# aexoden/snesimage

Measured on AMD Instinct MI355X. Metric: candidate palettes scored/sec, higher is better.
Workload: dtype f32

## Files before the change

snesimage_amd/csrc/kernels.hpp:

```cpp
#pragma once
#include "color.hpp"

namespace snes {

constexpr int kMaxScales = SSIM2_NUM_SCALES;
constexpr int kBlurRadius = 5;

SNES_HD long long idx_c4(int x, int y, int H) { return ((long long)(x >> 2) * H + y) * 4 + (x & 3); }
SNES_HD long long idx_r4(int x, int y, int W) { return ((long long)(y >> 2) * W + x) * 4 + (y & 3); }
SNES_HD long long idx_xt4(int x, int y, int H) { return ((((long long)(x >> 6) * (H >> 2)) + (y >> 2)) << 8) + ((x & 63) << 2) + (y & 3); }

struct BlurK {
    float n2[3];
    float d1[3];
};

struct Geom {
    int W, H, nscales;
    int sw[kMaxScales], sh[kMaxScales];
    int th[kMaxScales];
    long long off_xyb[kMaxScales], off_xybT[kMaxScales], off_hout[kMaxScales];
    long long cand_stride;
    long long src_off[kMaxScales];
};
// ... 318 lines not shown
            float v[3];
            const int o4 = down_odd_row(G, 5, by) - 2 * by;
            for (int c = 0; c < 3; c++) { float sum = 0.0f; sum += l4[c][0][0]; sum += l4[c][0][1]; sum += l4[c][o4][0]; sum += l4[c][o4][1]; v[c] = sum * 0.25f; }
            float X, Y, B;
            linear_to_positive_xyb(v[0], v[1], v[2], X, Y, B);
            if (by >= G.th[5]) X = Y = B = 0.0f;
            size_t ns = (size_t)WS * HS;
            float *o = wbase + (CAND ? G.off_xyb[5] : G.src_off[5]);
            float *oT = CAND ? (wbase + G.off_xybT[5]) : (P.workT + G.src_off[5]);
            o[(size_t)by * WS + bx] = X; o[ns + (size_t)by * WS + bx] = Y; o[2 * ns + (size_t)by * WS + bx] = B;
            oT[(size_t)bx * HS + by] = X; oT[ns + (size_t)bx * HS + by] = Y; oT[2 * ns + (size_t)bx * HS + by] = B;
        }
    }
#undef SNES_DOWN_LEVEL
}

__global__ __launch_bounds__(256) void k_source_scale0(const uint8_t *__restrict__ orig, const float *__restrict__ eotf, int W, int H,
                                                       float *__restrict__ lin0, float *__restrict__ img1, float *__restrict__ img1T) {
    int px = blockIdx.x * blockDim.x + threadIdx.x;
    if (px >= W * H) return;
    int x = px % W, y = px / W;
    uint32_t o = reinterpret_cast<const uint32_t *>(orig)[px];
    float r = eotf[o & 0xff], g = eotf[(o >> 8) & 0xff], b = eotf[(o >> 16) & 0xff];
    size_t n = (size_t)W * H;
    lin0[px] = r; lin0[n + px] = g; lin0[2 * n + px] = b;
    float X, Y, B;
    linear_to_positive_xyb(r, g, b, X, Y, B);
    img1[px] = X; img1[n + px] = Y; img1[2 * n + px] = B;
    size_t pt = (size_t)x * H + y;
    img1T[pt] = X; img1T[n + pt] = Y; img1T[2 * n + pt] = B;
}

__device__ __forceinline__ void maps_accumulate(double (&acc)[6], float m1, float sd1, float a1, double r1, float m2, float v22, float v12, float i2) {
    const float mu22 = m2 * m2, mu12 = m1 * m2;
    const float mu_diff = m1 - m2;
    const float num_m = fmaf(mu_diff, -mu_diff, 1.0f);
    const float num_s = fmaf(2.0f, v12 - mu12, SSIM2_C2);
    const float denom_s = sd1 + (v22 - mu22) + SSIM2_C2;
    double d = 1.0 - (double)((num_m * num_s) / denom_s);
    d = d > 0.0 ? d : 0.0;
    acc[0] += d;
    const double dd = d * d;
    acc[1] += dd * dd;
    const double d1 = ((double)fabsf(i2 - m2) - (double)a1) * r1;
    const double art = d1 > 0.0 ? d1 : 0.0;
    const double det = (-d1) > 0.0 ? (-d1) : 0.0;
    acc[2] += art;
    const double a2 = art * art;
    acc[3] += a2 * a2;
    acc[4] += det;
    const double l2 = det * det;
    acc[5] += l2 * l2;
}
__device__ __forceinline__ float source_sd1(float mu1, float sigma11) { const float mu11 = mu1 * mu1; return sigma11 - mu11; }
__device__ __forceinline__ float source_a1(float img1, float mu1) { return fabsf(img1 - mu1); }
__device__ __forceinline__ double source_r1(float a1) { return 1.0 / (1.0 + (double)a1); }
__global__ __launch_bounds__(256) void k_src_pad_rows(Geom G, float *__restrict__ sd1, double *__restrict__ r1) {
    const int s = (int)blockIdx.y;
    if (s >= G.nscales) return;
    const int W = G.sw[s], pad = G.sh[s] - G.th[s];
    const int n = 3 * W * pad;
    for (int i = (int)(blockIdx.x * blockDim.x + threadIdx.x); i < n; i += (int)(gridDim.x * blockDim.x)) {
        const int c = i / (W * pad), rem = i - c * (W * pad);
        const size_t idx = (size_t)G.src_off[s] + (size_t)c * W * G.sh[s] + (size_t)G.th[s] * W + rem;
        sd1[idx] = __builtin_nanf("");
        r1[idx] = 0.0;
    }
}

struct HParams {
    Geom G; BlurK K;
    int s, npairs, ncol, perceptual, use_maps, sub_size;
    const unsigned long long *packT; const float *pal_xyb; const float *cand_tab; const float *cand_lab; const float *labpxT;
    const float *in1T;
    const float *in2T;
    float *work;
    const uint8_t *mapsT; const uint8_t *tile_pal;
};

template <bool S0, bool PERCEPTUAL>
__global__ __launch_bounds__(256) void k_hpass(HParams P) {
    __shared__ __attribute__((aligned(16))) float buf[3][256][20];
    __shared__ float s_lut[3][256];
    const Geom &G = P.G;
    const int s = P.s;
    const int W = G.sw[s], H = G.sh[s];
    const int t = threadIdx.x;
    const int ppw = 256 / H;
    const int ql = t / H, y = t - ql * H;
    const int pair_raw = blockIdx.x * ppw + ql;
    const bool active = ql < ppw && pair_raw < P.npairs;
    const int pair = active ? pair_raw : 0;
    const int cand = pair / 3, ch = pair - cand * 3;
    const size_t ns = (size_t)W * H;

    float cand_v = 0.0f; uint32_t crgb = 0; Lab cl; cl.l = cl.a = cl.b = 0.0f; uint32_t cand_slot_ci = 0xffffffffu;
    if (S0) {
        for (int i = t; i < 3 * 256; i += 256) { int c = i >> 8, j = i & 255; s_lut[c][j] = (j < P.ncol + 2) ? P.pal_xyb[3 * j + c] : 0.0f; }
        cand_v = P.cand_tab[8 * (size_t)cand + 3 + ch];
        crgb = __float_as_uint(P.cand_tab[8 * (size_t)cand + 6]);
        cand_slot_ci = __float_as_uint(P.cand_tab[8 * (size_t)cand + 7]);
        if (PERCEPTUAL) { cl.l = P.cand_lab[3 * cand]; cl.a = P.cand_lab[3 * cand + 1]; cl.b = P.cand_lab[3 * cand + 2]; }
        __syncthreads();
    }
    const float *in1 = P.in1T + (size_t)ch * ns;
    const float *in2 = S0 ? nullptr : (P.in2T ? P.in2T + (size_t)ch * ns : P.work + (size_t)cand * G.cand_stride + G.off_xybT[s] + (size_t)ch * ns);
// ... 279 lines not shown
```

snesimage_amd/csrc/kernels_sparse.hpp:

```cpp
#pragma once
#include "kernels.hpp"

namespace snes {

constexpr int kGroupsTotal = 126;

struct CandMeta {
    int ngroups[kMaxScales];
    int xmin;
    int won;
    unsigned char glist[kGroupsTotal + 2];
    short gslot[kGroupsTotal];
    unsigned char gcb[kGroupsTotal];
};
__device__ __forceinline__ int item_k(unsigned int it) { return (int)(it >> 14); }
__device__ __forceinline__ int item_g(unsigned int it) { return (int)((it >> 8) & 63u); }
__device__ __forceinline__ int item_j(unsigned int it) { return (int)((it >> 2) & 63u); }
__device__ __forceinline__ int item_ch(unsigned int it) { return (int)(it & 3u); }
constexpr int kColBuckets = 4;
constexpr int kItemLists = kMaxScales * kColBuckets;

struct SparseGeom {
    long long off_lin[kMaxScales], off_xybC[kMaxScales], off_xybR[kMaxScales], off_hout[kMaxScales];
    long long cand_stride;
// ... 844 lines not shown
                if (P.perceptual && !is_base) {
                    const int px0 = y * W + (g << 2);
                    const uint32_t b4 = (P.bitmap[(size_t)k * (G.W * G.H / 32) + (px0 >> 5)] >> (px0 & 31)) & 0xfu;
                    c0 = (b4 & 1u) ? (uint32_t)P.ncol : (c_pa.x >> 24); c1 = (b4 & 2u) ? (uint32_t)P.ncol : (c_pa.z >> 24);
                    c2 = (b4 & 4u) ? (uint32_t)P.ncol : (c_pb.x >> 24); c3 = (b4 & 8u) ? (uint32_t)P.ncol : (c_pb.z >> 24);
                } else {
                    c0 = sparse_ci(c_pa.x, c_pa.y & never, crgb, (uint32_t)P.ncol); c1 = sparse_ci(c_pa.z, c_pa.w & never, crgb, (uint32_t)P.ncol);
                    c2 = sparse_ci(c_pb.x, c_pb.y & never, crgb, (uint32_t)P.ncol); c3 = sparse_ci(c_pb.z, c_pb.w & never, crgb, (uint32_t)P.ncol);
                }
                r2[u].x = c0 == (uint32_t)P.ncol ? cand_v : s_lut[ch][c0]; r2[u].y = c1 == (uint32_t)P.ncol ? cand_v : s_lut[ch][c1];
                r2[u].z = c2 == (uint32_t)P.ncol ? cand_v : s_lut[ch][c2]; r2[u].w = c3 == (uint32_t)P.ncol ? cand_v : s_lut[ch][c3];
            }
            const float v1[4] = {r1[u].x, r1[u].y, r1[u].z, r1[u].w}, v2[4] = {r2[u].x, r2[u].y, r2[u].z, r2[u].w};
            const float l1[4] = {r1[ua].z, r1[ua].w, r1[ub].x, r1[ub].y}, l2[4] = {r2[ua].z, r2[ua].w, r2[ub].x, r2[ub].y};
            float outp[3][4];
#pragma unroll
            for (int q = 0; q < 4; q++) {
                const float s0 = l2[q] + v2[q];
                const float s1 = (l2[q] * l2[q]) + (v2[q] * v2[q]);
                const float s2 = (l1[q] * l2[q]) + (v1[q] * v2[q]);
                if ((q & 1) == 0) { SNES_HSTEP(s0, sa[0], sb[0], outp[0][q]) SNES_HSTEP(s1, sa[1], sb[1], outp[1][q]) SNES_HSTEP(s2, sa[2], sb[2], outp[2][q]) }
                else { SNES_HSTEP(s0, sb[0], sa[0], outp[0][q]) SNES_HSTEP(s1, sb[1], sa[1], outp[1][q]) SNES_HSTEP(s2, sb[2], sa[2], outp[2][q]) }
            }
            if (g >= 1) {
#pragma unroll
                for (int p = 0; p < 3; p++) {
                    s_tr[p][lane * 5 + 0] = outp[p][0]; s_tr[p][lane * 5 + 1] = outp[p][1]; s_tr[p][lane * 5 + 2] = outp[p][2]; s_tr[p][lane * 5 + 3] = outp[p][3];
                }
                __syncthreads();
                const int x = ((g - 1) << 2) + li;
                const size_t o = ((size_t)(x >> 6) << 8) + ((size_t)(x & 63) << 2);
                if (valid) {
#pragma unroll
                    for (int p = 0; p < 3; p++) {
                        float4 v;
                        v.x = s_tr[p][(k4 + 0) * 5 + li]; v.y = s_tr[p][(k4 + 1) * 5 + li]; v.z = s_tr[p][(k4 + 2) * 5 + li]; v.w = s_tr[p][(k4 + 3) * 5 + li];
                        *reinterpret_cast<float4 *>(out + (size_t)p * 4 * W + o) = v;
                    }
                }
                __syncthreads();
            }
        }
    }
    }
}

template <bool UNI, int S0M, int BM>
__device__ __forceinline__ void sparse_v_body(const SparseParams &P, const int s) {
    __shared__ float s_lut[256];
    __shared__ short s_gslot[256];
    __shared__ __attribute__((aligned(16))) unsigned char s_raw[(2 + 3) * 3 * 256 * sizeof(float2)];
    float2 (*s_xy)[3][256] = reinterpret_cast<float2 (*)[3][256]>(s_raw);
    float2 (*s_zw)[3][256] = reinterpret_cast<float2 (*)[3][256]>(s_raw + 2 * 3 * 256 * sizeof(float2));
    double (*red)[6] = reinterpret_cast<double (*)[6]>(s_raw);
    static_assert(sizeof(s_raw) >= 256 * 6 * sizeof(double), "reduction scratch must fit the tail ring");
    const Geom &G = P.G;
    if (s >= G.nscales) return;
    const int W = G.sw[s], H = G.sh[s];
    const bool S0 = S0M == 2 ? s == 0 : S0M == 1;
    const int t = threadIdx.x;
    const int ppw = 256 / W;
    const bool is_base = BM == 2 ? P.is_base != 0 : BM == 1;
    const int npairs = is_base ? 3 : P.ncand * 3;
    if ((int)blockIdx.x * ppw >= npairs) return;
    const int ql = t / W, x = t - ql * W;
    const int pair_raw = blockIdx.x * ppw + ql;
    const bool active = pair_raw < npairs;
    const int pair = active ? pair_raw : 0;
    const int k = is_base ? P.base : P.k0 + (P.order ? P.order[pair / 3] : pair / 3), ch = pair % 3;
    if (S0) {
        s_lut[t] = (t < P.ncol + 2) ? P.pal_xyb[3 * t + ch] : 0.0f;
    }
    const size_t ns = (size_t)W * H;
    const int H4 = H >> 2;
    const CandMeta *M = P.meta + k;
    for (int i = t; i < ppw * H4; i += 256) {
        const int pr = blockIdx.x * ppw + i / H4;
        const int pq = (pr < npairs ? pr : 0) / 3;
        const int kk = is_base ? P.base : P.k0 + (P.order ? P.order[pq] : pq);
        s_gslot[i] = (P.meta + kk)->gslot[P.S.goff[s] + i % H4];
    }
    __syncthreads();
    const short *gslot = s_gslot + ql * H4;
    const int ng = M->ngroups[s];
    const int cmin = (M->xmin >> s) - 5;
    const bool skip = !is_base && (ng == 0 || x <= cmin);
    int gs = skip ? H4 + 1 : (is_base ? 0 : (int)M->glist[P.S.goff[s]]);
    if (UNI) {
        const int gs_pair = is_base ? 0 : (ng == 0 ? H4 + 1 : (int)M->glist[P.S.goff[s]]);
        gs = __builtin_amdgcn_readfirstlane(__all(skip) ? H4 + 1 : gs_pair);
    }
#define SNES_GSLOT(I) (UNI ? __builtin_amdgcn_readfirstlane((int)gslot[I]) : (int)gslot[I])
    const float cand_v = is_base ? 0.0f : P.cand_tab[8 * (size_t)k + 3 + ch];
    const uint32_t crgb = is_base ? 0u : __float_as_uint(P.cand_tab[8 * (size_t)k + 6]);
    const uint32_t never = is_base ? 0u : 0xffffffffu;
    const float *mine = P.store + (size_t)k * P.S.cand_stride;
    const float *basep = P.store + (size_t)P.base * P.S.cand_stride;
    const size_t hx = ((size_t)(x >> 6) << 6) + (size_t)(x & 63);
    const float4 *hb = reinterpret_cast<const float4 *>(basep + P.S.off_hout[s]) + (size_t)(ch * 3) * W + hx;
    const float4 *hm = reinterpret_cast<const float4 *>(mine + P.S.off_hout[s]) + (size_t)(ch * 3) * W + hx;
    const float4 *xb = S0 ? nullptr : reinterpret_cast<const float4 *>(basep + P.S.off_xybR[s]) + (size_t)ch * W + x;
    const float4 *xm = S0 ? nullptr : reinterpret_cast<const float4 *>(mine + P.S.off_xybR[s]) + (size_t)ch * W + x;
    const float4 *mu1 = reinterpret_cast<const float4 *>(P.mu1R4 + G.src_off[s] + (size_t)ch * ns) + x;
    const float4 *sd1 = reinterpret_cast<const float4 *>(P.sd1R4 + G.src_off[s] + (size_t)ch * ns) + x;
    const float4 *a1 = reinterpret_cast<const float4 *>(P.a1R4 + G.src_off[s] + (size_t)ch * ns) + x;
    const double2 *r1 = reinterpret_cast<const double2 *>(P.r1R4 + G.src_off[s] + (size_t)ch * ns) + 2 * (size_t)x;
    const uint4 *pk = S0 ? reinterpret_cast<const uint4 *>(P.packR4) + 2 * (size_t)x : nullptr;
    float *ckf = P.ckf + P.S.off_ckf[s] + (size_t)ch * (H4 + 2) * 18 * W + x;
    double *cka = P.cka + P.S.off_cka[s] + (size_t)ch * (H4 + 2) * 6 * W + x;

    const float n2_0 = P.K.n2[0], n2_1 = P.K.n2[1], n2_2 = P.K.n2[2];
    const float d1_0 = P.K.d1[0], d1_1 = P.K.d1[1], d1_2 = P.K.d1[2];
    float sa[3][3], sb[3][3];
    double acc[6];
    if (is_base) {
#pragma unroll
        for (int p = 0; p < 3; p++)
#pragma unroll
            for (int q = 0; q < 3; q++) { sa[p][q] = 0.0f; sb[p][q] = 0.0f; }
#pragma unroll
        for (int q = 0; q < 6; q++) acc[q] = 0.0;
    } else {
        const float *cf = ckf + (size_t)gs * 18 * W;
        const double *ca = cka + (size_t)gs * 6 * W;
#pragma unroll
        for (int p = 0; p < 3; p++)
#pragma unroll
            for (int q = 0; q < 3; q++) { sa[p][q] = cf[(size_t)(p * 6 + q) * W]; sb[p][q] = cf[(size_t)(p * 6 + 3 + q) * W]; }
#pragma unroll
        for (int q = 0; q < 6; q++) acc[q] = ca[(size_t)q * W];
    }
    const int W9 = 9 * W, W3 = 3 * W;
    auto hgroup = [&](int g) -> const float4 * {
        const int sl = SNES_GSLOT(g);
        return sl >= 0 ? hm + (uint32_t)__mul24(sl, W9) : hb + (uint32_t)__mul24(g, W9);
    };
    auto hload = [&](int g, int p) -> float4 { return hgroup(g)[(uint32_t)__mul24(p, W)]; };
    const float4 zero4 = make_float4(0.f, 0.f, 0.f, 0.f);
    float4 bufA[3], bufB[3];
#pragma unroll
    for (int p = 0; p < 3; p++) {
        float4 g1 = zero4, g2 = zero4, g3 = zero4;
        bufA[p] = zero4; bufB[p] = zero4;
        if (UNI ? gs <= H4 : !skip) {
            if (gs < H4) bufA[p] = hload(gs, p);
            if (gs - 1 >= 0) g1 = hload(gs - 1, p);
            if (gs - 2 >= 0) g2 = hload(gs - 2, p);
            if (gs - 3 >= 0) g3 = hload(gs - 3, p);
        }
        s_xy[1][p][t] = make_float2(g1.x, g1.y); s_zw[2][p][t] = make_float2(g1.z, g1.w);
        s_xy[0][p][t] = make_float2(g2.x, g2.y); s_zw[1][p][t] = make_float2(g2.z, g2.w);
        s_zw[0][p][t] = make_float2(g3.z, g3.w);
    }
    const int gm0 = gs >= 1 ? gs - 1 : 0;
    const float4 *p_m1 = mu1 + (uint32_t)__mul24(gm0, W), *p_sd1 = sd1 + (uint32_t)__mul24(gm0, W), *p_a1 = a1 + (uint32_t)__mul24(gm0, W);
    const double2 *p_r1 = r1 + 2u * (uint32_t)__mul24(gm0, W);
    const uint4 *p_pk = S0 ? pk + 2u * (uint32_t)__mul24(gm0, W) : nullptr;
    const uint32_t *bm = (S0 && P.perceptual && !is_base) ? P.bitmap + (size_t)k * (G.W * G.H / 32) : nullptr;
    float4 n_m1 = zero4, n_sd1 = zero4, n_a1 = zero4, n_x = zero4;
    double2 n_ra = make_double2(1.0, 1.0), n_rb = n_ra;
    uint4 n_pa = make_uint4(0, 0, 0, 0), n_pb = n_pa;
    float *ck_f = BM == 1 ? ckf + (size_t)gs * 18 * W : nullptr;
    double *ck_a = BM == 1 ? cka + (size_t)gs * 6 * W : nullptr;
#define SNES_VGROUP(U, CUR, NXT)                                                                                              \
    {                                                                                                                         \
        const int g = g0 + (U);                                                                                               \
        if (g > H4) break;                                                                                                    \
// ... 26 lines not shown
                if (S0) { n_pa = p_pk[0]; n_pb = p_pk[1]; p_pk += 2 * W; }                                                    \
                else n_x = xb[(uint32_t)__mul24(g, W3)];                                                                      \
            }                                                                                                                 \
        } else if (g >= 1) {                                                                                                  \
            c_m1 = *p_m1; c_sd1 = *p_sd1; c_a1 = *p_a1; c_ra = p_r1[0]; c_rb = p_r1[1];                                       \
            p_m1 += W; p_sd1 += W; p_a1 += W; p_r1 += 2 * W;                                                                  \
            if (S0) { c_pa = p_pk[0]; c_pb = p_pk[1]; p_pk += 2 * W; }                                                        \
            else { const int sl = SNES_GSLOT(g - 1); c_x = sl >= 0 ? xm[(uint32_t)__mul24(sl, W3)] : xb[(uint32_t)__mul24(g - 1, W3)]; } \
        }                                                                                                                     \
        float outp[3][4];                                                                                                     \
        _Pragma("unroll") for (int p = 0; p < 3; p++) {                                                                       \
            const float2 tz = s_zw[(U) % 3][p][t], tx = s_xy[(U) % 2][p][t];       \
            s_zw[(U) % 3][p][t] = make_float2(CUR[p].z, CUR[p].w);                                                            \
            s_xy[(U) % 2][p][t] = make_float2(CUR[p].x, CUR[p].y);                                                            \
            SNES_VSTEP(tz.x + CUR[p].x, sa[p], sb[p], outp[p][0])                                                             \
            SNES_VSTEP(tz.y + CUR[p].y, sb[p], sa[p], outp[p][1])                                                             \
            SNES_VSTEP(tx.x + CUR[p].z, sa[p], sb[p], outp[p][2])                                                             \
            SNES_VSTEP(tx.y + CUR[p].w, sb[p], sa[p], outp[p][3])                                                             \
        }                                                                                                                     \
        if (g >= 1) {                                                                                                         \
            float i2v[4] = {c_x.x, c_x.y, c_x.z, c_x.w};                                                                      \
            if (S0) {                                                                                                         \
                uint32_t c0, c1, c2, c3;                                                                                      \
                if (is_base || SNES_GSLOT(g - 1) < 0) {  \
                    c0 = c_pa.x >> 24; c1 = c_pa.z >> 24; c2 = c_pb.x >> 24; c3 = c_pb.z >> 24;                               \
                } else if (bm) {                                                       \
                    const int px0 = ((g - 1) << 2) * W + x;                                                                   \
                    c0 = won_bit(bm, px0) ? (uint32_t)P.ncol : (c_pa.x >> 24); c1 = won_bit(bm, px0 + W) ? (uint32_t)P.ncol : (c_pa.z >> 24);               \
                    c2 = won_bit(bm, px0 + 2 * W) ? (uint32_t)P.ncol : (c_pb.x >> 24); c3 = won_bit(bm, px0 + 3 * W) ? (uint32_t)P.ncol : (c_pb.z >> 24);   \
                } else {                                                                                                      \
                    c0 = sparse_ci(c_pa.x, c_pa.y & never, crgb, (uint32_t)P.ncol); c1 = sparse_ci(c_pa.z, c_pa.w & never, crgb, (uint32_t)P.ncol);         \
                    c2 = sparse_ci(c_pb.x, c_pb.y & never, crgb, (uint32_t)P.ncol); c3 = sparse_ci(c_pb.z, c_pb.w & never, crgb, (uint32_t)P.ncol);         \
                }                                                                                                             \
                i2v[0] = c0 == (uint32_t)P.ncol ? cand_v : s_lut[c0]; i2v[1] = c1 == (uint32_t)P.ncol ? cand_v : s_lut[c1];   \
                i2v[2] = c2 == (uint32_t)P.ncol ? cand_v : s_lut[c2]; i2v[3] = c3 == (uint32_t)P.ncol ? cand_v : s_lut[c3];   \
            }                                                                                                                 \
            const float m1v[4] = {c_m1.x, c_m1.y, c_m1.z, c_m1.w}, sd1v[4] = {c_sd1.x, c_sd1.y, c_sd1.z, c_sd1.w}, a1v[4] = {c_a1.x, c_a1.y, c_a1.z, c_a1.w}; \
            const double r1v[4] = {c_ra.x, c_ra.y, c_rb.x, c_rb.y};                                                           \
            _Pragma("unroll") for (int q = 0; q < 4; q++)                                                                     \
                maps_accumulate(acc, m1v[q], sd1v[q], a1v[q], r1v[q], outp[0][q], outp[1][q], outp[2][q], i2v[q]);            \
        }                                                                                                                     \
    }
    for (int g0 = gs; g0 <= H4; g0 += 6) {
        SNES_VGROUP(0, bufA, bufB) SNES_VGROUP(1, bufB, bufA) SNES_VGROUP(2, bufA, bufB)
        SNES_VGROUP(3, bufB, bufA) SNES_VGROUP(4, bufA, bufB) SNES_VGROUP(5, bufB, bufA)
    }
#undef SNES_VGROUP
#undef SNES_GSLOT
    if (is_base && active) {
        double *ca = cka + (size_t)(H4 + 1) * 6 * W;
#pragma unroll
        for (int q = 0; q < 6; q++) ca[(size_t)q * W] = acc[q];
    }
    __syncthreads();
#pragma unroll
    for (int q = 0; q < 6; q++) red[t][q] = active ? acc[q] : 0.0;
    __syncthreads();
    for (int stride = W >> 1; stride > 0; stride >>= 1) {
        if (x < stride) {
#pragma unroll
            for (int q = 0; q < 6; q++) red[t][q] += red[t + stride][q];
        }
        __syncthreads();
    }
    if (x == 0 && active) {
        double *o = P.part + (((size_t)k * G.nscales + s) * 3 + ch) * 6;
#pragma unroll
        for (int q = 0; q < 6; q++) o[q] = red[t][q];
    }
}
__global__ __launch_bounds__(256, 2) void k_sparse_v(SparseParams P) { sparse_v_body<false, 2, 2>(P, (int)blockIdx.y + P.s_first); }
__device__ __forceinline__ void sparse_v_base_body(const SparseParams &P) {
    const int s = (int)blockIdx.y;
    if (s >= P.G.nscales) return;
    if (P.G.sw[s] >= 64) sparse_v_body<true, 0, 1>(P, s);
    else sparse_v_body<false, 0, 1>(P, s);
}
#undef SNES_HSTEP
#undef SNES_VSTEP

__device__ __forceinline__ void build_plist_body(const unsigned long long *__restrict__ pack, int npx, uint4 *__restrict__ plist, int *__restrict__ count) {
    const int px = blockIdx.x * blockDim.x + threadIdx.x;
    unsigned long long w = 0;
    if (px < npx) w = pack[px];
    const uint32_t thr = (uint32_t)(w >> 32);
    const bool hit = thr != 0u;
    const unsigned long long m = __ballot(hit);
    if (m == 0ull) return;
    const int lane = threadIdx.x & 63, leader = __ffsll((long long)m) - 1;
    int base = 0;
    if (lane == leader) base = atomicAdd(count, __popcll(m));
    base = __shfl(base, leader);
    if (hit) plist[base + __popcll(m & ((1ull << lane) - 1ull))] = make_uint4((uint32_t)px, (uint32_t)w & 0x00ffffffu, thr, 0u);
}

__global__ __launch_bounds__(256) void k_remap_fill4(MapsParams P) {
    const int q = blockIdx.x * 256 + threadIdx.x;
    if (q * 4 >= P.npx) return;
    const uint4 a = reinterpret_cast<const uint4 *>(P.pack)[2 * (size_t)q], b = reinterpret_cast<const uint4 *>(P.pack)[2 * (size_t)q + 1];
    const uint32_t lo[4] = {a.x, a.z, b.x, b.z};
    uint32_t word = 0;
#pragma unroll
    for (int i = 0; i < 4; i++) {
        const uint32_t ci0 = lo[i] >> 24;
        word |= (ci0 == (uint32_t)P.ncol ? (uint32_t)P.si : (ci0 == (uint32_t)P.ncol + 1u ? 0u : ci0 % (uint32_t)P.sub_size)) << (8 * i);
    }
    const int c0 = blockIdx.y * kRemapCands;
    for (int cc = 0; cc < kRemapCands && c0 + cc < P.ncand; cc++) reinterpret_cast<uint32_t *>(P.maps + (size_t)(c0 + cc) * P.npx)[q] = word;
}
__global__ __launch_bounds__(256) void k_remap_won_lab(MapsParams P, const uint4 *__restrict__ plist, const int *__restrict__ plist_count) {
    __shared__ uint32_t s_queue[4][128];
    const int lane = threadIdx.x & 63, w = threadIdx.x >> 6;
    const int cand = (int)blockIdx.x;
    if (cand >= P.ncand) return;
    Lab cl; cl.l = P.cand_lab[3 * cand]; cl.a = P.cand_lab[3 * cand + 1]; cl.b = P.cand_lab[3 * cand + 2];
    const float cch = sqrtf(cl.a * cl.a + cl.b * cl.b);
    uint8_t *map = P.maps + (size_t)cand * P.npx;
    const int n = *plist_count;
    auto full_test = [&](int i) {
        const uint4 e = plist[i];
        Lab t; t.l = P.labpx[3 * (size_t)e.x]; t.a = P.labpx[3 * (size_t)e.x + 1]; t.b = P.labpx[3 * (size_t)e.x + 2];
// ... 59 lines not shown
```

snesimage_amd/csrc/kernels_sparse2.hpp:

```cpp
#pragma once
#include "kernels_sparse.hpp"
#include "kernels_fast.hpp"

namespace snes {

#define SNES_HSTEP(SUM, A, B, OUT)                                                   \
    {                                                                                \
        float o1_ = (SUM) * n2_0, o3_ = (SUM) * n2_1, o5_ = (SUM) * n2_2;            \
        o1_ = fmaf(-1.0f, B[0], o1_); o3_ = fmaf(-1.0f, B[1], o3_); o5_ = fmaf(-1.0f, B[2], o5_); \
        o1_ = fmaf(mp_0, A[0], o1_); o3_ = fmaf(mp_1, A[1], o3_); o5_ = fmaf(mp_2, A[2], o5_);    \
        B[0] = o1_; B[1] = o3_; B[2] = o5_;                                          \
        OUT = o1_ + o3_ + o5_;                                                       \
    }
#define SNES_VSTEP(SUM, A, B, OUT)                                                   \
    {                                                                                \
        float o1_ = fmaf(A[0], d1_0, B[0]), o3_ = fmaf(A[1], d1_1, B[1]), o5_ = fmaf(A[2], d1_2, B[2]); \
        o1_ = fmaf((SUM), n2_0, -o1_); o3_ = fmaf((SUM), n2_1, -o3_); o5_ = fmaf((SUM), n2_2, -o5_);    \
        B[0] = o1_; B[1] = o3_; B[2] = o5_;                                          \
        OUT = o1_ + o3_ + o5_;                                                       \
    }

struct H2Shared {
    __attribute__((aligned(16))) float out[16 * (4 * 32 + 4)];
    long long hbase[16], xbase[16];
// ... 280 lines not shown
                    const int im_ = 2 * m + half;                                                                             \
                    fv[m] = *reinterpret_cast<const float4 *>(s_out + im_ * ISTR + fl * 4);                                   \
                    fb[m] = (fp == 3) ? s_xbase[im_] : s_hbase[im_];                                                          \
                }                                                                                                             \
                _Pragma("unroll") for (int m = 0; m < 2; m++) {                                                               \
                    float *dst = (fb[m] >= 0 && fl < NP * 8) ? P.store + fb[m] + o_l : trash;                                 \
                    *reinterpret_cast<float4 *>(dst) = fv[m];                                                                 \
                }                                                                                                             \
                asm volatile("" ::: "memory");                                                                               \
            }                                                                                                                 \
        }
        { const int g = gs; SNES_H2Q_ITER(0, false, false) }
        for (int g0 = gs + 1; g0 <= G4; g0 += 6) {
            { const int g = g0; SNES_H2Q_ITER(1, true, false) }
            { const int g = g0 + 1; if (g > G4) break; SNES_H2Q_ITER(2, true, true) }
            { const int g = g0 + 2; if (g > G4) break; SNES_H2Q_ITER(3, true, false) }
            { const int g = g0 + 3; if (g > G4) break; SNES_H2Q_ITER(4, true, true) }
            { const int g = g0 + 4; if (g > G4) break; SNES_H2Q_ITER(5, true, false) }
            { const int g = g0 + 5; if (g > G4) break; SNES_H2Q_ITER(6, true, true) }
        }
#undef SNES_H2Q_ITER
    }
}
template <bool BASE>
__device__ __forceinline__ void sparse_h2q_dispatch(const SparseParams &P, const int list, const int bx, const int gx) {
    const int s = list / kColBuckets;
    if (s >= P.G.nscales || P.G.sw[s] < 64 || (list % kColBuckets) >= (P.G.sw[s] >> 6)) return;
    __shared__ H2Shared sh;
    if (s == 0) sparse_h2q_body<true, BASE>(P, list, bx, gx, sh); else sparse_h2q_body<false, BASE>(P, list, bx, gx, sh);
}

__device__ __forceinline__ int uni(int v) { return __builtin_amdgcn_readfirstlane(v); }
template <typename T> __device__ __forceinline__ T ld_at(const void *sbase, uint32_t voff) { return *reinterpret_cast<const T *>(reinterpret_cast<const char *>(sbase) + voff); }
typedef __amdgpu_buffer_rsrc_t rsrc_t;
typedef unsigned int u32x4 __attribute__((ext_vector_type(4)));
__device__ __forceinline__ rsrc_t make_rsrc(const void *p) {
    const unsigned long long a = (unsigned long long)p;
    const unsigned long long u = ((unsigned long long)(uint32_t)__builtin_amdgcn_readfirstlane((int)(a >> 32)) << 32) | (uint32_t)__builtin_amdgcn_readfirstlane((int)a);
    return __builtin_amdgcn_make_buffer_rsrc(reinterpret_cast<void *>(u), 0, 0x7fffffff, 0x00020000);
}
__device__ __forceinline__ float4 buf_ld4(rsrc_t r, uint32_t voff, uint32_t soff) {
    const u32x4 v = __builtin_amdgcn_raw_buffer_load_b128(r, (int)voff, (int)soff, 0);
    return make_float4(__uint_as_float(v.x), __uint_as_float(v.y), __uint_as_float(v.z), __uint_as_float(v.w));
}
__device__ __forceinline__ double2 buf_ld2d(rsrc_t r, uint32_t voff, uint32_t soff) {
    const u32x4 v = __builtin_amdgcn_raw_buffer_load_b128(r, (int)voff, (int)soff, 0);
    return make_double2(__hiloint2double((int)v.y, (int)v.x), __hiloint2double((int)v.w, (int)v.z));
}

template <bool BASE>
__device__ __forceinline__ void sparse_v2_body(const SparseParams &P, const int s, const int bx) {
    __shared__ short s_slot[4][64];
    __shared__ __attribute__((aligned(16))) unsigned char s_raw[(2 + 3) * 3 * 256 * sizeof(float2)];
    double (*red)[6] = reinterpret_cast<double (*)[6]>(s_raw);
    static_assert(sizeof(s_raw) >= 256 * 6 * sizeof(double), "reduction scratch must fit the tail ring");
    const Geom &G = P.G;
    const int W = uni(G.sw[s]), H = uni(G.sh[s]), H4 = H >> 2;
    const int t = threadIdx.x, lane = t & 63;
    const int wv = uni(t >> 6);
    const int wpp = W >> 6, ppw = 4 / wpp;
    const int npairs = BASE ? 3 : P.ncand * 3;
    if (bx * ppw >= npairs) return;
    const int ql = wv / wpp, xw = (wv - ql * wpp) << 6;
    const int pair_raw = bx * ppw + ql;
    const bool active = pair_raw < npairs;
    const int pair = active ? pair_raw : 0;
    const int ch = BASE ? pair : pair / P.ncand, ci = BASE ? 0 : pair - ch * P.ncand;
    const int k = BASE ? P.base : uni(P.k0 + (P.order ? P.order[ci] : ci));
    const CandMeta *M = P.meta + k;
    int gs;
    {
        const int g = lane;
        short sl = -1;
        if (!BASE && g < H4) { sl = M->gslot[P.S.goff[s] + g]; if (sl >= 0 && ((int)M->gcb[P.S.goff[s] + g] << 6) > xw) sl = -1; }
        s_slot[wv][lane] = sl;
        const unsigned long long own = __ballot(sl >= 0);
        gs = BASE ? 0 : uni(own ? __ffsll((long long)own) - 1 : H4 + 1);
    }
    __syncthreads();

    const size_t ns = (size_t)W * H;
    const float *store_k = P.store + (size_t)k * P.S.cand_stride, *store_b = P.store + (size_t)P.base * P.S.cand_stride;
    const rsrc_t h_own = make_rsrc(store_k + P.S.off_hout[s] + (size_t)(ch * 3) * 4 * W + ((size_t)(xw >> 6) << 8));
    const rsrc_t h_b = make_rsrc(store_b + P.S.off_hout[s] + (size_t)(ch * 3) * 4 * W + ((size_t)(xw >> 6) << 8));
    const rsrc_t h_zero = make_rsrc(P.zeros);
    const rsrc_t x_own = make_rsrc(store_k + P.S.off_xybR[s] + (size_t)ch * 4 * W + (size_t)xw * 4);
    const rsrc_t x_b = make_rsrc(store_b + P.S.off_xybR[s] + (size_t)ch * 4 * W + (size_t)xw * 4);
    const rsrc_t m1_b = make_rsrc(P.mu1R4 + G.src_off[s] + (size_t)ch * ns + (size_t)xw * 4);
    const rsrc_t sd1_b = make_rsrc(P.sd1R4 + G.src_off[s] + (size_t)ch * ns + (size_t)xw * 4);
    const rsrc_t a1_b = make_rsrc(P.a1R4 + G.src_off[s] + (size_t)ch * ns + (size_t)xw * 4);
    const rsrc_t r1_b = make_rsrc(P.r1R4 + G.src_off[s] + (size_t)ch * ns + (size_t)xw * 4);
    const uint32_t l4 = (uint32_t)lane << 2, l8 = (uint32_t)lane << 3, l16 = (uint32_t)lane << 4, l32 = (uint32_t)lane << 5;
    const uint32_t W16 = (uint32_t)W * 16u;

    const float n2_0 = P.K.n2[0], n2_1 = P.K.n2[1], n2_2 = P.K.n2[2];
    const float d1_0 = P.K.d1[0], d1_1 = P.K.d1[1], d1_2 = P.K.d1[2];
    float sa[3][3], sb[3][3];
    double acc[6];
    float *ck_f = P.ckf + P.S.off_ckf[s] + ((size_t)ch * (H4 + 2)) * 18 * W + xw + lane;
    double *ck_a = P.cka + P.S.off_cka[s] + ((size_t)ch * (H4 + 2)) * 6 * W + xw + lane;
    if (BASE) {
#pragma unroll
        for (int p = 0; p < 3; p++)
#pragma unroll
            for (int q = 0; q < 3; q++) { sa[p][q] = 0.0f; sb[p][q] = 0.0f; }
#pragma unroll
        for (int q = 0; q < 6; q++) acc[q] = 0.0;
    } else {
        const float *cf = P.ckf + P.S.off_ckf[s] + ((size_t)ch * (H4 + 2) + gs) * 18 * W + xw;
        const double *ca = P.cka + P.S.off_cka[s] + ((size_t)ch * (H4 + 2) + gs) * 6 * W + xw;
#pragma unroll
        for (int p = 0; p < 3; p++)
#pragma unroll
            for (int q = 0; q < 3; q++) { sa[p][q] = ld_at<float>(cf + (size_t)(p * 6 + q) * W, l4); sb[p][q] = ld_at<float>(cf + (size_t)(p * 6 + 3 + q) * W, l4); }
#pragma unroll
        for (int q = 0; q < 6; q++) acc[q] = ld_at<double>(ca + (size_t)q * W, l8);
    }
#define SNES_HLOAD(GG, DST)                                                                                                   \
    {                                                                                                                         \
        const int gg_ = (GG);                                                                                                 \
        const bool below_ = gg_ >= H4;                                                                                        \
        const int sl_ = uni((int)s_slot[wv][below_ ? 0 : gg_]);                                                               \
        const rsrc_t r_ = below_ ? h_zero : (sl_ >= 0 ? h_own : h_b);                                                         \
        const uint32_t so_ = below_ ? 0u : (uint32_t)(sl_ >= 0 ? sl_ : gg_) * 9u * W16;                                       \
        DST[0] = buf_ld4(r_, l16, so_); DST[1] = buf_ld4(r_, l16, so_ + W16); DST[2] = buf_ld4(r_, l16, so_ + 2u * W16);      \
    }
    const float4 zero4 = make_float4(0.f, 0.f, 0.f, 0.f);
    float2 *ring_xy = reinterpret_cast<float2 *>(s_raw) + t;
    float2 *ring_zw = reinterpret_cast<float2 *>(s_raw + 2 * 3 * 256 * sizeof(float2)) + t;
    float4 bufA[3], bufB[3];
    float4 t1[3] = {zero4, zero4, zero4}, t2[3] = {zero4, zero4, zero4}, t3[3] = {zero4, zero4, zero4};
#pragma unroll
    for (int p = 0; p < 3; p++) { bufA[p] = zero4; bufB[p] = zero4; }
    if (gs <= H4) {
        if (gs < H4) SNES_HLOAD(gs, bufA)
        if (gs - 1 >= 0) SNES_HLOAD(gs - 1, t1)
        if (gs - 2 >= 0) SNES_HLOAD(gs - 2, t2)
        if (gs - 3 >= 0) SNES_HLOAD(gs - 3, t3)
    }
#pragma unroll
    for (int p = 0; p < 3; p++) {
        const float4 g1 = t1[p], g2 = t2[p], g3 = t3[p];
        ring_xy[(1 * 3 + p) * 256] = make_float2(g1.x, g1.y); ring_zw[(2 * 3 + p) * 256] = make_float2(g1.z, g1.w);
        ring_xy[(0 * 3 + p) * 256] = make_float2(g2.x, g2.y); ring_zw[(1 * 3 + p) * 256] = make_float2(g2.z, g2.w);
        ring_zw[(0 * 3 + p) * 256] = make_float2(g3.z, g3.w);
    }
    int r2 = 0, r3 = 0;
#define SNES_V2GROUP(CUR, NXT)                                                                                                \
    {                                                                                                                         \
        if (BASE && active) {                                                                                   \
            _Pragma("unroll") for (int p = 0; p < 3; p++)                                                                     \
                _Pragma("unroll") for (int q = 0; q < 3; q++) { ck_f[(size_t)(p * 6 + q) * W] = sa[p][q]; ck_f[(size_t)(p * 6 + 3 + q) * W] = sb[p][q]; } \
            _Pragma("unroll") for (int q = 0; q < 6; q++) ck_a[(size_t)q * W] = acc[q];                                       \
            ck_f += (size_t)18 * W; ck_a += (size_t)6 * W;                                                                    \
        }                                                                                                                     \
        SNES_HLOAD(g + 1, NXT)                                                                                                \
                \
        float4 c_m1, c_sd1, c_a1, c_x;                                                                                        \
        double2 c_ra, c_rb;                                                                                                   \
        {                                                                                                                     \
            const int gm = g >= 1 ? g - 1 : 0;                                                                                \
            const uint32_t go = (uint32_t)gm * W16;                                                                           \
            c_m1 = buf_ld4(m1_b, l16, go); c_sd1 = buf_ld4(sd1_b, l16, go); c_a1 = buf_ld4(a1_b, l16, go);                    \
            c_ra = buf_ld2d(r1_b, l32, 2u * go); c_rb = buf_ld2d(r1_b, l32 + 16u, 2u * go);                                   \
            const int sl = uni((int)s_slot[wv][gm]);                                                                          \
            c_x = buf_ld4(sl >= 0 ? x_own : x_b, l16, (uint32_t)(sl >= 0 ? sl : gm) * 3u * W16);                              \
        }                                                                                                                     \
        float outp[3][4];                                                                                                     \
        _Pragma("unroll") for (int p = 0; p < 3; p++) {                                                                       \
            float2 *pz = ring_zw + (r3 * 3 + p) * 256, *px = ring_xy + (r2 * 3 + p) * 256;                                    \
            const float2 tz = *pz, tx = *px;                                       \
            *pz = make_float2(CUR[p].z, CUR[p].w);                                                                            \
            *px = make_float2(CUR[p].x, CUR[p].y);                                                                            \
            SNES_VSTEP(tz.x + CUR[p].x, sa[p], sb[p], outp[p][0])                                                             \
            SNES_VSTEP(tz.y + CUR[p].y, sb[p], sa[p], outp[p][1])                                                             \
            SNES_VSTEP(tx.x + CUR[p].z, sa[p], sb[p], outp[p][2])                                                             \
            SNES_VSTEP(tx.y + CUR[p].w, sb[p], sa[p], outp[p][3])                                                             \
        }                                                                                                                     \
          \
        asm volatile("" : "+v"(c_a1.x), "+v"(c_a1.y), "+v"(c_a1.z), "+v"(c_a1.w));                                            \
        if (g >= 1) {                                                                                                         \
            const float m1v[4] = {c_m1.x, c_m1.y, c_m1.z, c_m1.w}, sd1v[4] = {c_sd1.x, c_sd1.y, c_sd1.z, c_sd1.w};              \
            const float a1v[4] = {c_a1.x, c_a1.y, c_a1.z, c_a1.w}, i2v[4] = {c_x.x, c_x.y, c_x.z, c_x.w};                     \
            const double r1v[4] = {c_ra.x, c_ra.y, c_rb.x, c_rb.y};                                                           \
            _Pragma("unroll") for (int q = 0; q < 4; q++)                                                                     \
                maps_accumulate(acc, m1v[q], sd1v[q], a1v[q], r1v[q], outp[0][q], outp[1][q], outp[2][q], i2v[q]);            \
        }                                                                                                                     \
        r2 ^= 1; r3 = r3 == 2 ? 0 : r3 + 1;                                                                                   \
    }
    for (int g = gs; g <= H4; g++) {
        SNES_V2GROUP(bufA, bufB)
        g++;
        if (g > H4) break;
        SNES_V2GROUP(bufB, bufA)
    }
#undef SNES_V2GROUP
#undef SNES_HLOAD
    if (BASE && active) {
#pragma unroll
        for (int q = 0; q < 6; q++) ck_a[(size_t)q * W] = acc[q];
    }
    __syncthreads();
#pragma unroll
    for (int q = 0; q < 6; q++) red[t][q] = active ? acc[q] : 0.0;
    __syncthreads();
    const int xp = t & (W - 1);
    for (int stride = W >> 1; stride > 0; stride >>= 1) {
        if (xp < stride) {
#pragma unroll
            for (int q = 0; q < 6; q++) red[t][q] += red[t + stride][q];
        }
        __syncthreads();
    }
    if (xp == 0 && active) {
        double *o = P.part + (((size_t)k * G.nscales + s) * 3 + ch) * 6;
#pragma unroll
        for (int q = 0; q < 6; q++) o[q] = red[t][q];
    }
}
__device__ __forceinline__ void lds_barrier() { asm volatile("s_waitcnt lgkmcnt(0)\n\ts_barrier" ::: "memory"); }
__device__ __forceinline__ void sparse_v2_base_split_body(const SparseParams &P, const int s, const int ch, const int cb) {
    __shared__ __attribute__((aligned(16))) float s_x[2][3][64][4];
    const Geom &G = P.G;
    const int W = uni(G.sw[s]), H = uni(G.sh[s]), H4 = H >> 2;
    const int lane = threadIdx.x & 63;
    const bool is_r = uni((int)(threadIdx.x >> 6)) == 0;
    const int xw = cb << 6;
    const size_t ns = (size_t)W * H;
    const float *store_b = P.store + (size_t)P.base * P.S.cand_stride;
    const uint32_t l16 = (uint32_t)lane << 4, l32 = (uint32_t)lane << 5;
    const uint32_t W16 = (uint32_t)W * 16u;
    const float4 zero4 = make_float4(0.f, 0.f, 0.f, 0.f);
    if (is_r) {
        const rsrc_t h_b = make_rsrc(store_b + P.S.off_hout[s] + (size_t)(ch * 3) * 4 * W + ((size_t)(xw >> 6) << 8));
        const rsrc_t h_zero = make_rsrc(P.zeros);
        const float n2_0 = P.K.n2[0], n2_1 = P.K.n2[1], n2_2 = P.K.n2[2];
        const float d1_0 = P.K.d1[0], d1_1 = P.K.d1[1], d1_2 = P.K.d1[2];
        float sa[3][3], sb[3][3];
#pragma unroll
        for (int p = 0; p < 3; p++)
#pragma unroll
            for (int q = 0; q < 3; q++) { sa[p][q] = 0.0f; sb[p][q] = 0.0f; }
        float *ck_f = P.ckf + P.S.off_ckf[s] + ((size_t)ch * (H4 + 2)) * 18 * W + xw + lane;
        float4 ring[3][3];
        float4 nxt[3];
#pragma unroll
        for (int p = 0; p < 3; p++) { ring[p][0] = zero4; ring[p][1] = zero4; ring[p][2] = zero4; }
#define SNES_V2S_HLOAD(GG, DST) { const int gg_ = (GG); const bool below_ = gg_ >= H4; const rsrc_t r_ = below_ ? h_zero : h_b; const uint32_t so_ = below_ ? 0u : (uint32_t)gg_ * 9u * W16; \
            DST[0] = buf_ld4(r_, l16, so_); DST[1] = buf_ld4(r_, l16, so_ + W16); DST[2] = buf_ld4(r_, l16, so_ + 2u * W16); }
        SNES_V2S_HLOAD(0, nxt)
#define SNES_V2S_RITER(T)                                                                                   \
        {                                                                                                                     \
            constexpr int u_ = (T) % 3, ux_ = ((T) + 1) % 3;                                                                  \
            _Pragma("unroll") for (int p = 0; p < 3; p++)                                                                     \
                _Pragma("unroll") for (int q = 0; q < 3; q++) { ck_f[(size_t)(p * 6 + q) * W] = sa[p][q]; ck_f[(size_t)(p * 6 + 3 + q) * W] = sb[p][q]; } \
            ck_f += (size_t)18 * W;                                                                                           \
            float4 cur[3] = {nxt[0], nxt[1], nxt[2]};                                                                         \
            SNES_V2S_HLOAD(g + 1, nxt)                                                                                        \
            _Pragma("unroll") for (int p = 0; p < 3; p++) {                                                                   \
                const float4 tz = ring[p][u_], tx = ring[p][ux_];        \
                float4 o;                                                                                                     \
                SNES_VSTEP(tz.z + cur[p].x, sa[p], sb[p], o.x)                                                                \
                SNES_VSTEP(tz.w + cur[p].y, sb[p], sa[p], o.y)                                                                \
                SNES_VSTEP(tx.x + cur[p].z, sa[p], sb[p], o.z)                                                                \
                SNES_VSTEP(tx.y + cur[p].w, sb[p], sa[p], o.w)                                                                \
                ring[p][u_] = cur[p];                                                                                         \
                *reinterpret_cast<float4 *>(&s_x[g & 1][p][lane][0]) = o;                                                     \
            }                                                                                                                 \
        }
        for (int g0 = 0; g0 <= H4 + 1; g0 += 3) {
// ... 69 lines not shown
```

Measured before the change: 2.907 million.

## Replace LDS tree reduction with shuffle/DPP pooling and skip fully-cached waves

Replaces the per-block shared-memory tree reduction of the six f64 SSIM accumulators, which needed a barrier per level, with a cross-wave LDS step followed by intra-wave shuffles and DPP row ops. It also adds an early path where, if every lane in the wave is skipped, the final accumulators are loaded directly from the checkpoint buffer instead of running the blur/accumulate loop. This cuts barriers and LDS traffic in the vertical sparse kernels. It risks changing floating-point summation order and relies on DPP semantics for 64-bit values split into halves. Profiling helper scripts are added as well.

```diff
diff --git a/profiles/isa_summary.py b/profiles/isa_summary.py
--- /dev/null
+++ b/profiles/isa_summary.py
@@ -0,0 +1,23 @@
+#!/usr/bin/env python3
+import re
+import sys
+
+
+def main():
+    text = open(sys.argv[1]).read()
+    for want in sys.argv[2:]:
+        m = re.search(r"^(_ZN4snes%d%sE\w*):[^\n]*\n(.*?)^\s*\.amdhsa_kernel \1\n.*?; Kernel info:\n(.*?)^\s*\.text" % (len(want), re.escape(want)), text, re.S | re.M)
+        if not m:
+            print("%s: not found" % want)
+            continue
+        code, info = m.group(2), m.group(3)
+        ins = [l.strip() for l in code.splitlines() if l.startswith("\t") and not l.strip().startswith((".", ";"))]
+        f = lambda k: re.search(r"; %s: (\d+)" % k, info).group(1)
+        n = lambda rx: sum(bool(re.match(rx, i)) for i in ins)
+        print("%s: VGPRs %s, LDS %s B, occupancy %s, scratch %s B | instructions %d, s_barrier %d, vector-memory loads %d, stores %d, scratch accesses %d, LDS ops %d, binary64 VALU %d" % (
+            want, f("NumVgprs"), f("LDSByteSize"), f("Occupancy"), f("ScratchSize"), len(ins), n(r"s_barrier"), n(r"(global|buffer|flat)_load"),
+            n(r"(global|buffer|flat)_store"), n(r"scratch_"), n(r"ds_"), n(r"v_\w+_f64")))
+
+
+if __name__ == "__main__":
+    main()
diff --git a/profiles/rocprof_tables.py b/profiles/rocprof_tables.py
--- /dev/null
+++ b/profiles/rocprof_tables.py
@@ -0,0 +1,46 @@
+#!/usr/bin/env python3
+import csv
+import glob
+import os
+import sys
+from collections import defaultdict
+
+
+def find(d, suffix):
+    hits = sorted(glob.glob(os.path.join(d, "**", "*" + suffix), recursive=True))
+    if not hits:
+        raise SystemExit("no *%s under %s" % (suffix, d))
+    return hits[0]
+
+
+def short(name):
+    name = name.replace("snes::", "")
+    return name.split("(")[0][:60]
+
+
+def stats(d, top=30):
+    rows = list(csv.DictReader(open(find(d, "kernel_stats.csv"))))
+    tot = sum(float(r["TotalDurationNs"]) for r in rows)
+    print("%-60s %7s %12s %10s %10s %6s" % ("kernel", "calls", "total_us", "avg_us", "max_us", "%"))
+    for r in sorted(rows, key=lambda r: -float(r["TotalDurationNs"]))[:top]:
+        print("%-60s %7d %12.1f %10.1f %10.1f %6.2f" % (short(r["Name"]), int(r["Calls"]), float(r["TotalDurationNs"]) / 1e3, float(r["AverageNs"]) / 1e3,
+                                                         float(r["MaxNs"]) / 1e3, 100.0 * float(r["TotalDurationNs"]) / tot))
+    print("%-60s %7s %12.1f" % ("all kernels", "", tot / 1e3))
+
+
+def pmc(d, top=30):
+    disp = {}
+    for r in csv.DictReader(open(find(d, "counter_collection.csv"))):
+        k = disp.setdefault(r["Dispatch_Id"], {"name": short(r["Kernel_Name"]), "us": (float(r["End_Timestamp"]) - float(r["Start_Timestamp"])) / 1e3})
+        k[r["Counter_Name"]] = k.get(r["Counter_Name"], 0.0) + float(r["Counter_Value"])
+    agg = defaultdict(lambda: [0, 0.0, 0.0, 0.0])
+    for k in disp.values():
+        a = agg[k["name"]]
+        a[0] += 1; a[1] += k["us"]; a[2] += k.get("SQ_WAVES", 0.0); a[3] += k.get("SQ_INSTS_VALU", 0.0)
+    print("%-60s %6s %10s %10s %10s" % ("kernel (alone on the chip)", "n", "avg_us", "waves", "VALU/wave"))
+    for name, a in sorted(agg.items(), key=lambda kv: -kv[1][1])[:top]:
+        print("%-60s %6d %10.1f %10.0f %10.1f" % (name, a[0], a[1] / a[0], a[2] / a[0], a[3] / a[2] if a[2] else 0.0))
+
+
+if __name__ == "__main__":
+    {"stats": stats, "pmc": pmc}[sys.argv[1]](sys.argv[2])
diff --git a/snesimage_amd/csrc/kernels.hpp b/snesimage_amd/csrc/kernels.hpp
--- a/snesimage_amd/csrc/kernels.hpp
+++ b/snesimage_amd/csrc/kernels.hpp
@@ -394,6 +394,57 @@
     const double l2 = det * det;
     acc[5] += l2 * l2;
 }
+template <int CTRL>
+__device__ __forceinline__ double dpp_row_f64(const double v) {
+    const int lo = __builtin_amdgcn_update_dpp(0, __double2loint(v), CTRL, 0xf, 0xf, false);
+    const int hi = __builtin_amdgcn_update_dpp(0, __double2hiint(v), CTRL, 0xf, 0xf, false);
+    return __hiloint2double(hi, lo);
+}
+__device__ __forceinline__ void pool_reduce(double (&acc)[6], double *const scratch, const int t, const int W) {
+    if (W > 64) {
+        const int wq = (t >> 6) & ((W >> 6) - 1);
+        if (wq != 0) {
+#pragma unroll
+            for (int q = 0; q < 6; q++) scratch[q * 256 + t] = acc[q];
+        }
+        __syncthreads();
+        if (wq != 0) return;
+        if (W == 256) {
+#pragma unroll
+            for (int q = 0; q < 6; q++) {
+                const double w1 = scratch[q * 256 + t + 64], w2 = scratch[q * 256 + t + 128], w3 = scratch[q * 256 + t + 192];
+                acc[q] = (acc[q] + w2) + (w1 + w3);
+            }
+        } else {
+#pragma unroll
+            for (int q = 0; q < 6; q++) acc[q] += scratch[q * 256 + t + 64];
+        }
+    }
+    if (W >= 64) {
+#pragma unroll
+        for (int q = 0; q < 6; q++) acc[q] += __shfl_down(acc[q], 32);
+    }
+    if (W >= 32) {
+#pragma unroll
+        for (int q = 0; q < 6; q++) acc[q] += __shfl_down(acc[q], 16);
+    }
+    if (W >= 16) {
+#pragma unroll
+        for (int q = 0; q < 6; q++) acc[q] += dpp_row_f64<0x108>(acc[q]);
+    }
+    if (W >= 8) {
+#pragma unroll
+        for (int q = 0; q < 6; q++) acc[q] += dpp_row_f64<0x104>(acc[q]);
+    }
+    if (W >= 4) {
+#pragma unroll
+        for (int q = 0; q < 6; q++) acc[q] += dpp_row_f64<0x102>(acc[q]);
+    }
+    if (W >= 2) {
+#pragma unroll
+        for (int q = 0; q < 6; q++) acc[q] += dpp_row_f64<0x101>(acc[q]);
+    }
+}
 __device__ __forceinline__ float source_sd1(float mu1, float sigma11) { const float mu11 = mu1 * mu1; return sigma11 - mu11; }
 __device__ __forceinline__ float source_a1(float img1, float mu1) { return fabsf(img1 - mu1); }
 __device__ __forceinline__ double source_r1(float a1) { return 1.0 / (1.0 + (double)a1); }
diff --git a/snesimage_amd/csrc/kernels_sparse.hpp b/snesimage_amd/csrc/kernels_sparse.hpp
--- a/snesimage_amd/csrc/kernels_sparse.hpp
+++ b/snesimage_amd/csrc/kernels_sparse.hpp
@@ -920,7 +920,7 @@
     __shared__ __attribute__((aligned(16))) unsigned char s_raw[(2 + 3) * 3 * 256 * sizeof(float2)];
     float2 (*s_xy)[3][256] = reinterpret_cast<float2 (*)[3][256]>(s_raw);
     float2 (*s_zw)[3][256] = reinterpret_cast<float2 (*)[3][256]>(s_raw + 2 * 3 * 256 * sizeof(float2));
-    double (*red)[6] = reinterpret_cast<double (*)[6]>(s_raw);
+    double *const red = reinterpret_cast<double *>(s_raw);
     static_assert(sizeof(s_raw) >= 256 * 6 * sizeof(double), "reduction scratch must fit the tail ring");
     const Geom &G = P.G;
     if (s >= G.nscales) return;
@@ -958,6 +958,12 @@
         const int gs_pair = is_base ? 0 : (ng == 0 ? H4 + 1 : (int)M->glist[P.S.goff[s]]);
         gs = __builtin_amdgcn_readfirstlane(__all(skip) ? H4 + 1 : gs_pair);
     }
+    double acc[6];
+    if (!is_base && __all(skip)) {
+        const double *ca = P.cka + P.S.off_cka[s] + ((size_t)ch * (H4 + 2) + (H4 + 1)) * 6 * W + x;
+#pragma unroll
+        for (int q = 0; q < 6; q++) acc[q] = ca[(size_t)q * W];
+    } else {
 #define SNES_GSLOT(I) (UNI ? __builtin_amdgcn_readfirstlane((int)gslot[I]) : (int)gslot[I])
     const float cand_v = is_base ? 0.0f : P.cand_tab[8 * (size_t)k + 3 + ch];
     const uint32_t crgb = is_base ? 0u : __float_as_uint(P.cand_tab[8 * (size_t)k + 6]);
@@ -980,7 +986,6 @@
     const float n2_0 = P.K.n2[0], n2_1 = P.K.n2[1], n2_2 = P.K.n2[2];
     const float d1_0 = P.K.d1[0], d1_1 = P.K.d1[1], d1_2 = P.K.d1[2];
     float sa[3][3], sb[3][3];
-    double acc[6];
     if (is_base) {
 #pragma unroll
         for (int p = 0; p < 3; p++)
@@ -1113,21 +1118,12 @@
 #pragma unroll
         for (int q = 0; q < 6; q++) ca[(size_t)q * W] = acc[q];
     }
-    __syncthreads();
-#pragma unroll
-    for (int q = 0; q < 6; q++) red[t][q] = active ? acc[q] : 0.0;
-    __syncthreads();
-    for (int stride = W >> 1; stride > 0; stride >>= 1) {
-        if (x < stride) {
-#pragma unroll
-            for (int q = 0; q < 6; q++) red[t][q] += red[t + stride][q];
-        }
-        __syncthreads();
-    }
+    }
+    pool_reduce(acc, red, t, W);
     if (x == 0 && active) {
         double *o = P.part + (((size_t)k * G.nscales + s) * 3 + ch) * 6;
 #pragma unroll
-        for (int q = 0; q < 6; q++) o[q] = red[t][q];
+        for (int q = 0; q < 6; q++) o[q] = acc[q];
     }
 }
 __global__ __launch_bounds__(256, 2) void k_sparse_v(SparseParams P) { sparse_v_body<false, 2, 2>(P, (int)blockIdx.y + P.s_first); }
diff --git a/snesimage_amd/csrc/kernels_sparse2.hpp b/snesimage_amd/csrc/kernels_sparse2.hpp
--- a/snesimage_amd/csrc/kernels_sparse2.hpp
+++ b/snesimage_amd/csrc/kernels_sparse2.hpp
@@ -356,7 +356,6 @@
 __device__ __forceinline__ void sparse_v2_body(const SparseParams &P, const int s, const int bx) {
     __shared__ short s_slot[4][64];
     __shared__ __attribute__((aligned(16))) unsigned char s_raw[(2 + 3) * 3 * 256 * sizeof(float2)];
-    double (*red)[6] = reinterpret_cast<double (*)[6]>(s_raw);
     static_assert(sizeof(s_raw) >= 256 * 6 * sizeof(double), "reduction scratch must fit the tail ring");
     const Geom &G = P.G;
     const int W = uni(G.sw[s]), H = uni(G.sh[s]), H4 = H >> 2;
@@ -381,8 +380,15 @@
         const unsigned long long own = __ballot(sl >= 0);
         gs = BASE ? 0 : uni(own ? __ffsll((long long)own) - 1 : H4 + 1);
     }
-    __syncthreads();
-
+    lds_order();
+
+    double acc[6];
+    double *const red = reinterpret_cast<double *>(s_raw);
+    if (!BASE && gs > H4) {
+        const double *ca = P.cka + P.S.off_cka[s] + ((size_t)ch * (H4 + 2) + (H4 + 1)) * 6 * W + xw;
+#pragma unroll
+        for (int q = 0; q < 6; q++) acc[q] = ld_at<double>(ca + (size_t)q * W, (uint32_t)lane << 3);
+    } else {
     const size_t ns = (size_t)W * H;
     const float *store_k = P.store + (size_t)k * P.S.cand_stride, *store_b = P.store + (size_t)P.base * P.S.cand_stride;
     const rsrc_t h_own = make_rsrc(store_k + P.S.off_hout[s] + (size_t)(ch * 3) * 4 * W + ((size_t)(xw >> 6) << 8));
@@ -400,7 +406,6 @@
     const float n2_0 = P.K.n2[0], n2_1 = P.K.n2[1], n2_2 = P.K.n2[2];
     const float d1_0 = P.K.d1[0], d1_1 = P.K.d1[1], d1_2 = P.K.d1[2];
     float sa[3][3], sb[3][3];
-    double acc[6];
     float *ck_f = P.ckf + P.S.off_ckf[s] + ((size_t)ch * (H4 + 2)) * 18 * W + xw + lane;
     double *ck_a = P.cka + P.S.off_cka[s] + ((size_t)ch * (H4 + 2)) * 6 * W + xw + lane;
     if (BASE) {
@@ -504,22 +509,12 @@
 #pragma unroll
         for (int q = 0; q < 6; q++) ck_a[(size_t)q * W] = acc[q];
     }
-    __syncthreads();
-#pragma unroll
-    for (int q = 0; q < 6; q++) red[t][q] = active ? acc[q] : 0.0;
-    __syncthreads();
-    const int xp = t & (W - 1);
-    for (int stride = W >> 1; stride > 0; stride >>= 1) {
-        if (xp < stride) {
-#pragma unroll
-            for (int q = 0; q < 6; q++) red[t][q] += red[t + stride][q];
-        }
-        __syncthreads();
-    }
-    if (xp == 0 && active) {
+    }
+    pool_reduce(acc, red, t, W);
+    if ((t & (W - 1)) == 0 && active) {
         double *o = P.part + (((size_t)k * G.nscales + s) * 3 + ch) * 6;
 #pragma unroll
-        for (int q = 0; q < 6; q++) o[q] = red[t][q];
+        for (int q = 0; q < 6; q++) o[q] = acc[q];
     }
 }
 __device__ __forceinline__ void lds_barrier() { asm volatile("s_waitcnt lgkmcnt(0)\n\ts_barrier" ::: "memory"); }
```

After: 2.934 million, median of 6. Within noise of the previous version (+0.9%).
